# yhz0/SQLP

Measured on AMD Instinct MI355X. Metric: stage-2 subproblems/sec + cut-gen HBM GB/s on STORM, higher is better.
Workload: dtype f64

## Files before the change

### sqlp_amd/csrc/api.hip

```cpp
#include <hip/hip_runtime.h>
#include <algorithm>
#include <cmath>
#include <cstdarg>
#include <cstdio>
#include <cstdlib>
#include <cstring>
#include <string>
#include <vector>
#include <map>
#include <memory>
#include <thread>
#include <chrono>
#include "twosd_internal.h"
#include "twosd_ctx.h"

using namespace twosd;

static thread_local std::string g_err;

int twosd::fail(int code, const char *fmt, ...) {
    char buf[1024];
    va_list ap;
    va_start(ap, fmt);
    vsnprintf(buf, sizeof buf, fmt, ap);
// ... 203 lines not shown
}
template <typename T>
static int upload_big(twosd_ctx *c, T **d, const std::vector<T> &h) {
    return upload_big(c, d, h.data(), h.size());
}

static int reserve_selection(twosd_ctx *c, int P, int records) {
    int rc;
    if ((size_t)std::max(records, 1) > c->sel_code_cap) {
        dfree(c->d_sel_code);
        if ((rc = dalloc(&c->d_sel_code, 2 * (size_t)std::max(records, 1)))) return rc;
        c->sel_code_cap = std::max(records, 1);
    }
    if ((rc = dev_reserve(c, &c->d_sel_end, (size_t)P)) || (rc = dev_reserve(c, &c->d_sel_cinf, (size_t)P))) return rc;
    c->sel_cap_total = records;
    return TWOSD_OK;
}

template <typename T>
static int upload(T **d, const std::vector<T> &h) {
    int rc = dalloc(d, std::max<size_t>(h.size(), 1));
    if (rc) return rc;
    if (!h.empty()) HIPCHK(hipMemcpy(*d, h.data(), sizeof(T) * h.size(), hipMemcpyHostToDevice));
    return TWOSD_OK;
}

static void free_template(twosd_ctx *c) {
    dfree(c->d_colptr); dfree(c->d_rowidx); dfree(c->d_val); dfree(c->d_q); dfree(c->d_btype);
    dfree(c->d_fixedmask); dfree(c->d_ubmask);
    dfree(c->d_hb0); dfree(c->d_basic0);
    dfree(c->d_xbase); dfree(c->d_queue); dfree(c->d_lpstats);
    dfree(c->d_obj); dfree(c->d_pi); dfree(c->d_pi_rep); dfree(c->d_y); dfree(c->d_status); dfree(c->d_iters); dfree(c->d_ops); dfree(c->d_etan);
    dfree(c->d_dvtmp);
    dfree(c->d_bnnz); dfree(c->d_sel_cinf); dfree(c->d_sel_ptr); dfree(c->d_sel_code); c->sel_code_cap = 0; dfree(c->d_head_out); dfree(c->d_pool_pick); dfree(c->d_cpick); dfree(c->d_order); dfree(c->d_sort_tmp);
    dfree(c->d_cand); dfree(c->d_sel_key); dfree(c->d_sel_pkey); dfree(c->d_sel_ppick); c->sel_pcap = 0; c->key_cap = 0; c->pool_l1 = c->pool_ncand = 0; c->order_cap = 0; c->sort_tmp_bytes = 0; c->head_cap = 0; c->pick_cap = 0; c->pool.clear();
    dfree(c->d_dist_kind); dfree(c->d_dist_off); dfree(c->d_dist_val); dfree(c->d_dist_prob); dfree(c->d_dist_p0);
    dfree(c->d_dist_p1); dfree(c->d_dist_tmpl); c->has_dist = false;
    dfree(c->d_kslot); dfree(c->d_kix); dfree(c->d_kv); dfree(c->d_kcoef); c->k_valid = false;
    dfree(c->d_sel_end); dfree(c->d_kp); dfree(c->d_ke); dfree(c->d_kraw); dfree(c->d_xaux); c->xaux_cap = 0; c->sel_cap_total = 0;
    dfree(c->d_d0); dfree(c->d_eidx); dfree(c->d_evals); dfree(c->d_stamps);
    dfree(c->d_wcp); dfree(c->d_wcc); dfree(c->d_wcv); dfree(c->d_bcp); dfree(c->d_bci); dfree(c->d_bcv);
    dfree(c->d_brptr); dfree(c->d_brcol); dfree(c->d_brval);
    c->earena_slots = 0; c->earena_cap = 0;
    for (auto &e : c->epis) { dfree(e.d_dv); dfree(e.d_w); }
    c->epis.clear();
    c->out_cap = 0; c->dvtmp_cap = 0;
    dvs_free(c);
    cut_free(c);
    vkey_free(c);
    c->dcap.clear();
    dfree(c->d_vkey); c->vkey_cap = 0;
    dfree(c->d_bkey); c->bkey_cap = 0;
    dfree(c->d_refresh_sel); c->refresh_sel_cap = 0; c->box_epi = -1;
    dfree(c->d_eo_pb); dfree(c->d_eo_K); dfree(c->d_eo_off); dfree(c->d_eo_etap); dfree(c->d_eo_etaoff);
    dfree(c->d_eo_eidx); dfree(c->d_eo_evals); dfree(c->d_eo_used); c->eo_rows = c->eo_cap = 0; c->eo_kmax = 0;
    dfree(c->d_pg_scrow); dfree(c->d_pg_scoff); dfree(c->d_pg_scval); dfree(c->d_pg_ival); dfree(c->d_pg_irow); dfree(c->d_pg_ioff); dfree(c->d_pg_amax); dfree(c->d_pg_d0p); dfree(c->d_pg_cnt); dfree(c->d_pg_tot);
    dfree(c->d_pg_valid); dfree(c->d_pg_head0); dfree(c->d_pg_map); dfree(c->d_pg_off); dfree(c->d_pg_pos);
    dfree(c->d_rt_pack); dfree(c->d_gs_heads); dfree(c->d_gs_cnt); dfree(c->d_gs_tot); dfree(c->d_gs_valid);
    dfree(c->d_gs_irow); dfree(c->d_gs_ioff); dfree(c->d_gs_ival);
    if (c->d_gs_seg) { hipFree(c->d_gs_seg); c->d_gs_seg = nullptr; c->gs_seg_cap = 0; }
    c->rt_epi = -1; c->rt_nown = -1; c->rt_trained = false;
    if (c->pool_hb) { hipHostFree(c->pool_hb); c->pool_hb = nullptr; c->pool_hb_cap = 0; }
    c->has_template = c->has_basis = false;
}

extern "C" int twosd_destroy(twosd_ctx *c) {
    if (!c) return TWOSD_OK;
// ... 1907 lines not shown
            const size_t need = list ? (size_t)NL : (size_t)N;
            if (need > c->head_cap) {
                if ((rc = dalloc(&c->d_head_out, need * m))) return rc;
                c->head_cap = need;
            }
            H.head_out = c->d_head_out;
        }
        H.pi_by_pos = list ? 1 : 0;
        H.status = c->d_status; H.iters = c->d_iters; H.ops = c->d_ops; H.etan = c->d_etan;
        if (!c->d_lpstats && (rc = dalloc(&c->d_lpstats, 6))) return rc;
        if (!list) HIPCHK(hipMemsetAsync(c->d_lpstats + 5, 0, sizeof(unsigned long long), c->stream));
        H.retries = list ? nullptr : c->d_lpstats + 5;
        if (!c->d_stamps) {
            if ((rc = dalloc(&c->d_stamps, 16))) return rc;
            HIPCHK(hipMemset(c->d_stamps, 0, sizeof(unsigned long long) * 16));
        }
        H.stamps = c->d_stamps;
        H.npool = (int)c->pool.size();
        H.bnnz = c->d_bnnz;
        if (c->want_head && !list) {
            if ((size_t)N > c->head_cap) {
                if ((rc = dalloc(&c->d_head_out, (size_t)N * m))) return rc;
                c->head_cap = N;
            }
            H.head_out = c->d_head_out;
        }
        if (H.npool > 1) {
            if (!list && (size_t)N > c->pick_cap) {
                if ((rc = dalloc(&c->d_pool_pick, (size_t)N))) return rc;
                c->pick_cap = N;
            }
            H.pool_pick = c->d_pool_pick;
        }
        HIPCHK(hipEventRecord(c->ev[0], c->stream));
        if (list) {
            H.order = o.d_list;
        } else if (H.npool > 1) {
            if ((rc = select_pool(c, d_dv, N, c->d_pool_pick, 0))) return rc;
            H.order = c->d_order;
        }
        HIPCHK(hipEventRecord(c->ev[2], c->stream));
        HIPCHK(launch_hyper(R, CH, H, nblocks, hyper_lds_bytes(R, CH, kmax, c->k), c->stream));
        HIPCHK(hipEventRecord(c->ev[1], c->stream));
        HIPCHK(hipStreamSynchronize(c->stream));
        float ms = 0, ms_sel = 0;
        hipEventElapsedTime(&ms, c->ev[2], c->ev[1]);
        hipEventElapsedTime(&ms_sel, c->ev[0], c->ev[2]);
        c->t_us[0] = 1e3 * ms;
        c->t_us[4] = 1e3 * ms_sel;
        if (list) return TWOSD_OK;
        c->last_lp_N = N;
        c->last_lp_blocks = nblocks;
        c->last_ops_width = 1;
        return TWOSD_OK;
    }
}

__global__ void __launch_bounds__(256) lp_stats_kernel(int N, const int *__restrict__ its, const long long *__restrict__ ops,
                                                      const int *__restrict__ st, const int *__restrict__ etan,
                                                      unsigned long long *out) {
    __shared__ unsigned long long red[4][5];
    unsigned long long a = 0, b = 0, d = 0, e = 0;
    unsigned long long mx = 0;
    for (int s = blockIdx.x * blockDim.x + threadIdx.x; s < N; s += gridDim.x * blockDim.x) {
        a += (unsigned long long)its[s];
        b += (unsigned long long)ops[s];
        mx = its[s] > (int)mx ? (unsigned long long)its[s] : mx;
        d += st[s] != TWOSD_LP_OPTIMAL;
        e += (unsigned long long)etan[s];
    }
    for (int o = 32; o > 0; o >>= 1) {
        a += __shfl_down(a, o);
        b += __shfl_down(b, o);
        d += __shfl_down(d, o);
// ... 345 lines not shown
```

### sqlp_amd/csrc/lp_hyper.hip

```cpp
#include <hip/hip_runtime.h>
#include <math.h>
#include <type_traits>
#include "twosd_internal.h"
#include "wave_ops.h"

namespace twosd {

#define HTOL_P 1e-9
#define HTOL_D 1e-9
#define HTOL_PIV 1e-9
#define HPI_ZERO 1e-12


#ifdef TWOSD_STAMPS
#define STAMP_DECL unsigned long long st_acc[10] = {0, 0, 0, 0, 0, 0, 0, 0, 0, 0}; \
    unsigned long long st_last = __builtin_amdgcn_s_memtime();
#define STAMP(i)                                                      \
    {                                                                 \
        const unsigned long long t_ = __builtin_amdgcn_s_memtime();   \
        st_acc[i] += t_ - st_last;                                    \
        st_last = t_;                                                 \
    }
#define STAMP_FLUSH                                                                         \
    if (lane == 0 && P.stamps)                                                              \
// ... 152 lines not shown
    using Mask = typename std::conditional<(C > 32), uint64_t, uint32_t>::type;
    const int lane = threadIdx.x & 63;
    const int wid = threadIdx.x >> 6;
    constexpr int MP = 64 * R;
    constexpr int UD = 128 * R > 64 * C ? 128 * R : 64 * C;
    const int kmaxp = (P.kmax + 3) & ~3;
    const int ncol = P.n + P.m;
    char *slice = reinterpret_cast<char *>(lds_raw) + (size_t)wid * hyper_slice_bytes(R, C, P.kmax, P.k);
    double *ut = reinterpret_cast<double *>(slice);
    double *rho = ut + MP;
    double *alpha = ut;
    double *dvl = ut + UD;
    double *lstv = dvl + ((P.k + 1) & ~1);
    int *lsti = reinterpret_cast<int *>(lstv + 64);
    int *smark = lsti + 64;
    unsigned short *etap = reinterpret_cast<unsigned short *>(smark + 64);
    int *etaoff = reinterpret_cast<int *>(etap + kmaxp);

    const int m = P.m, n = P.n;
    const int slot_id = blockIdx.x * kWavesPerBlock + wid;
    int *eidx = P.eidx + (size_t)slot_id * P.ecap;
    double *evals = P.evals + (size_t)slot_id * P.ecap;
    const uint64_t fixedm = CP.fixedmask[lane];
    const uint64_t ubm = CP.ubmask[lane];

    for (int j = lane; j < UD; j += 64) ut[j] = 0.0;
    smark[lane] = 0;
    h_wave_sync();
    STAMP_DECL

    const int G = CP.qgroups;
    const int g0 = blockIdx.x % G;
    int gt = 0;
    auto group_of = [&](int gi) { return g0 + gi < G ? g0 + gi : g0 + gi - G; };
    auto claim_sync = [&]() -> int {
        for (; gt < G; ++gt) {
            const int g = group_of(gt);
            const int lo = (int)(((long long)P.N * g) / G), hi = (int)(((long long)P.N * (g + 1)) / G);
            int t = 0;
            if (lane == 0) t = atomicAdd(CP.queue + g * kQueueStride, 1);
            t = __builtin_amdgcn_readfirstlane(__shfl(t, 0));
            if (lo + t < hi) return lo + t;
        }
        return -1;
    };
    int q_nx = claim_sync();
    int s_nx = q_nx < 0 ? -1 : (CP.order ? __builtin_amdgcn_readfirstlane(CP.order[q_nx]) : q_nx);
    int pb_nx = (s_nx >= 0 && CP.npool > 1) ? __builtin_amdgcn_readfirstlane(CP.pool_pick[s_nx]) : 0;
    auto dv_fill = [&](int sn) {
        const double *dvs = CP.dv + (size_t)sn * P.k;
        for (int e = lane; e < P.k; e += 64) dvl[e] = CP.kcoef[e] * dvs[e];
    };
    const bool dv_pf = P.k <= 128;
    if (s_nx >= 0 && dv_pf) dv_fill(s_nx);
    for (;;) {
        if (q_nx < 0) break;
        const int qpos = q_nx;
        int s = s_nx;
        int pb = pb_nx;
        int t_claim = 0;
        if (lane == 0 && gt < G) t_claim = atomicAdd(CP.queue + group_of(gt) * kQueueStride, 1);

        if (!dv_pf) dv_fill(s);
        h_wave_sync();
        int lnx = lane;
        asm volatile("" : "+v"(lnx));
        double xB[R];
        float wd[R];
        int hb[R];
        double d[C];
        uint64_t bmask;
        const int *brptr, *bcp;
        int K = 0, it = 0, status = TWOSD_LP_OPTIMAL;
        int eoff = 0;
        unsigned nops = 0;
        for (int attempt = 0; attempt < 2; ++attempt) {
        {
            const auto *A = h_args();
            const int ln = lnx;
            brptr = A->brptr + (size_t)pb * (MP + 1);
            bcp = A->bcp + (size_t)pb * (MP + 1);
            const double *xb = A->xbase + (size_t)pb * MP;
            const double *kv = A->kv;
            const int *kix = A->kix;
            const int ksv = ln <= R ? A->kslot[pb * (R + 1) + ln] : 0;
            int eb[R], len[R];
            int w = 0;
#pragma unroll
            for (int t = 0; t < R; ++t) {
                eb[t] = __builtin_amdgcn_readlane(ksv, t);
                len[t] = __builtin_amdgcn_readlane(ksv, t + 1) - eb[t];
                w = len[t] > w ? len[t] : w;
                xB[t] = xb[64 * t + ln];
                hb[t] = A->hb0[(size_t)pb * MP + 64 * t + ln];
                wd[t] = 1.0f;
            }
            nops += (unsigned)(__builtin_amdgcn_readlane(ksv, R) - eb[0]) * 64u;
            for (int u0 = 0; u0 < w; u0 += XU) {
                double kvv[XU][R];
                int kiv[XU][R];
#pragma unroll
                for (int uu = 0; uu < XU; ++uu)
#pragma unroll
                    for (int t = 0; t < R; ++t) {
                        const int u = u0 + uu;
                        kvv[uu][t] = 0.0;
                        kiv[uu][t] = 0;
                        if (u < len[t]) {
                            kvv[uu][t] = kv[(size_t)(eb[t] + u) * 64 + ln];
                            kiv[uu][t] = kix[(size_t)(eb[t] + u) * 64 + ln];
                        }
                    }
#pragma unroll
                for (int uu = 0; uu < XU; ++uu)
#pragma unroll
                    for (int t = 0; t < R; ++t)
                        if (u0 + uu < len[t]) xB[t] = fma(kvv[uu][t], dvl[kiv[uu][t]], xB[t]);
            }
            uint64_t ub = ubm;
            asm volatile("" : "+v"(ub));
#pragma unroll
            for (int c = 0; c < C; ++c)
                d[c] = h_flip(A->d0[(size_t)pb * 64 * C + 64 * c + ln], ((ub >> c) & 1) << 63);
            bmask = A->basic0[pb * 64 + ln];
        }
        K = 0; status = TWOSD_LP_OPTIMAL; eoff = 0;
        if (lane == 0) etaoff[0] = 0;
        h_wave_sync();
        if (attempt == 0) {
            if (gt < G) {
                const int g = group_of(gt);
                const int hi = (int)(((long long)P.N * (g + 1)) / G), lo = (int)(((long long)P.N * g) / G);
                const int t = __builtin_amdgcn_readfirstlane(__shfl(t_claim, 0));
                if (lo + t < hi) q_nx = lo + t;
                else { ++gt; q_nx = claim_sync(); }
            } else {
                q_nx = -1;
            }
            if (q_nx >= 0) s_nx = CP.order ? CP.order[q_nx] : q_nx;
        }
        STAMP(0)

        auto eta_group = [&](int t0, int dir, int (&gi)[EG], double (&gv)[EG], int (&gn)[EG], int (&go)[EG]) {
#pragma unroll
            for (int g = 0; g < EG; ++g) {
                const int tt = t0 + dir * g;
                const bool ok = (tt >= 0) & (tt < K);
                const int tc = ok ? tt : 0;
                const int o0 = etaoff[tc], o1 = etaoff[tc + 1];
                go[g] = ok ? o0 : 0;
                gn[g] = ok ? o1 - o0 : 0;
                const bool mine = lane < gn[g];
                const int at = mine ? go[g] + lane : 0;
                const int ix = eidx[at];
                const double vx = evals[at];
                gi[g] = mine ? ix : 0;
                gv[g] = mine ? vx : 0.0;
            }
        };
        for (;;) {
            double bnum = 0.0, bden = 1.0, bdel = 0.0;
            int br = 0x7fffffff;
#pragma unroll
            for (int t = 0; t < R; ++t) {
                const int bt = hb[t] & 3;
                const bool inf = (hb[t] >= 0) & (((xB[t] < -HTOL_P) & (bt != BT_G)) | ((xB[t] > HTOL_P) & ((bt & 1) != 0)));
                if (__builtin_amdgcn_ballot_w64(inf) != 0 && inf) {
                    const double dl = xB[t];
                    const double num = dl * dl, den = (double)wd[t];
                    if (num * bden > bnum * den) { bnum = num; bden = den; br = 64 * t + lane; bdel = dl; }
                }
            }
            const ArgBest1 lr = warg_max1(bnum / bden, br, bdel);
// ... 8 lines not shown
                int p0 = 0, len = 0;
                double gr = 0.0;
                if (lane < nb) {
                    const int gi = lsti[lane];
                    gr = lstv[lane];
                    p0 = P.wcp[gi];
                    len = P.wcp[gi + 1] - p0;
                    alpha[n + gi] = P.btype[n + gi] == BT_G ? -gr : gr;
                }
                nops += h_seg_scatter(p0, len, gr, P.wcc, P.wcv, alpha, smark, lane) + nb;
                h_wave_sync();
            };
            int rp0 = 0, rlen = 65;
            if (K == 0) {
                rp0 = __builtin_amdgcn_readfirstlane(brptr[r]);
                rlen = __builtin_amdgcn_readfirstlane(brptr[r + 1]) - rp0;
            }
            if (rlen <= 64) {
                int gi = 0;
                double gr = 0.0;
                if (lane < rlen) {
                    gi = P.brcol[rp0 + lane];
                    gr = P.brval[rp0 + lane];
                }
                const uint64_t nzm = __ballot(gr != 0.0);
                if (gr != 0.0) {
                    const int pos = h_prefix_count(nzm);
                    lsti[pos] = gi;
                    lstv[pos] = gr;
                }
                nops += rlen;
                if (nzm != 0) price_batch(__popcll(nzm));
            } else {
                if (lane == (r & 63)) ut[r] = 1.0;
                h_wave_sync();
                const int gp0 = lane <= K ? (lane == 0 ? r : (int)etap[K - lane]) : -1;
                int bp0 = 0, bp1 = 0;
                if (gp0 >= 0) {
                    bp0 = brptr[gp0];
                    bp1 = brptr[gp0 + 1];
                }
                {
                    auto apply = [&](int tg, const int (&gi)[EG], const double (&gv)[EG], const int (&gn)[EG], const int (&go)[EG]) {
#pragma unroll
                        for (int g = 0; g < EG; ++g) {
                            const int tt = tg - g;
                            if (tt < 0) break;
                            const double ug = gv[g] != 0.0 ? ut[gi[g]] : 0.0;
                            if (gn[g] <= 64 && __builtin_amdgcn_ballot_w64(ug != 0.0) == 0) {
                                nops += gn[g];
                                continue;
                            }
                            double acc = ug * gv[g];
                            for (int e = 64 + lane; e < gn[g]; e += 64) acc = fma(ut[eidx[go[g] + e]], evals[go[g] + e], acc);
                            acc = wsum(acc);
                            nops += gn[g];
                            if (lane == 0) ut[etap[tt]] = acc;
                            h_wave_sync();
                        }
                    };
                    int ai[EG], an[EG], ao[EG], bi[EG], bn[EG], bo[EG];
                    double av[EG], bv[EG];
                    if (K <= 2 * EG) {
                        for (int tg = K - 1; tg >= 0; tg -= EG) {
                            eta_group(tg, -1, ai, av, an, ao);
                            apply(tg, ai, av, an, ao);
                        }
// ... 36 lines not shown
#pragma unroll
                for (int t = 0; t < R; ++t) rv[t] = rho[64 * t + lane];
                h_wave_sync();
#pragma unroll
                for (int t = 0; t < R; ++t) rho[64 * t + lane] = 0.0;
                h_wave_sync();
                uint64_t mk[R];
                int tot = 0;
#pragma unroll
                for (int t = 0; t < R; ++t) {
                    mk[t] = __ballot(rv[t] != 0.0);
                    tot += __popcll(mk[t]);
                }
                for (int b0 = 0; b0 < tot; b0 += 64) {
                    int base = -b0;
#pragma unroll
                    for (int t = 0; t < R; ++t) {
                        const int pos = base + h_prefix_count(mk[t]);
                        if (rv[t] != 0.0 && pos >= 0 && pos < 64) {
                            lsti[pos] = 64 * t + lane;
                            lstv[pos] = rv[t];
                        }
                        base += __popcll(mk[t]);
                    }
                    price_batch(tot - b0 < 64 ? tot - b0 : 64);
                }
            }
            h_wave_sync();
            STAMP(4)

            const uint64_t sgm = delta > 0 ? 0ull : (1ull << 63);
            const Mask cand = (Mask)~(bmask | fixedm);
            double bnu = INFINITY, bde = 1.0;
            Mask elm = 0, sel = 0, snz = 0;
            double apf = alpha[lane];
#pragma unroll
            for (int c = 0; c < C; ++c) {
                const double av = apf;
                if (c + 1 < C) apf = alpha[64 * (c + 1) + lane];
                const double a = h_flip(av, sgm);
                const bool el = (((cand >> c) & 1) != 0) & (a > HTOL_PIV);
                snz = h_uniform(snz | ((Mask)(__builtin_amdgcn_ballot_w64(av != 0.0) != 0) << c));
                if (__builtin_amdgcn_ballot_w64(el) != 0) {
                    sel |= (Mask)1 << c;
                    const double nu = d[c] + HTOL_D;
                    const bool better = el & (nu * bde < bnu * a);
                    bnu = better ? nu : bnu;
                    bde = better ? a : bde;
                    elm |= (Mask)el << c;
                }
                __builtin_amdgcn_sched_barrier(0);
            }
            const double thmax = wmin(bnu / bde);
            if (thmax == INFINITY) {
                status = TWOSD_LP_INFEASIBLE;
                h_wave_sync();
#pragma unroll
                for (int c = 0; c < C; ++c) alpha[64 * c + lane] = 0.0;
                break;
            }
            double bA = 0.0, bD = 0.0;
            int bq = 0x7fffffff;
            apf = alpha[lane];
#pragma unroll
            for (int c = 0; c < C; ++c) {
                const double av = apf;
// ... 160 lines not shown
            ++K;
            const int lh = h_get_row_i<R>(hb, r);
            const int leaving = lh >> 2;
            {
                const int ls = __builtin_amdgcn_readfirstlane(leaving >> 6), qs = __builtin_amdgcn_readfirstlane(q >> 6);
                const double dlv = (delta > 0) == ((lh & 3) == BT_G) ? thetaD : -thetaD;
                const bool lme = lane == (leaving & 63), qme = lane == (q & 63);
                H_SLOT_SWITCH(ls, C, {
                    double v = lme ? dlv : d[SL];
                    asm volatile("" : "+v"(v));
                    d[SL] = v;
                })
                H_SLOT_SWITCH(qs, C, {
                    double v = qme ? 0.0 : d[SL];
                    asm volatile("" : "+v"(v));
                    d[SL] = v;
                })
                if (lme) bmask &= ~(1ull << ls);
                if (qme) bmask |= 1ull << qs;
                {
                    const int nh = q * 4 + (int)P.btype[q];
                    const bool rme = lane == (r & 63);
                    H_SLOT_SWITCH(__builtin_amdgcn_readfirstlane(r >> 6), R, {
                        int v = rme ? nh : hb[SL];
                        asm volatile("" : "+v"(v));
                        hb[SL] = v;
                    })
                }
            }
            ++it;
            h_wave_sync();
            STAMP(8)
        }
        if (attempt == 0 && q_nx >= 0) {
            s_nx = __builtin_amdgcn_readfirstlane(s_nx);
            if (CP.npool > 1) pb_nx = CP.pool_pick[s_nx];
        }
        if (status == TWOSD_LP_OPTIMAL || pb == 0 || !CP.retry) break;
        if (lane == 0 && CP.retries) atomicAdd(CP.retries, 1ull);
        pb = 0;
        }
        double dvn0 = 0.0, dvn1 = 0.0, kcn0 = 0.0, kcn1 = 0.0;
        if (dv_pf && q_nx >= 0) {
            const auto *A = h_args();
            const double *dvs = A->dv + (size_t)s_nx * P.k;
            if (lane < P.k) { dvn0 = dvs[lane]; kcn0 = A->kcoef[lane]; }
            if (lane + 64 < P.k) { dvn1 = dvs[lane + 64]; kcn1 = A->kcoef[lane + 64]; }
        }

        double objv = NAN;
        if (status == TWOSD_LP_OPTIMAL) {
            const double *qc = CP.q;
            double qv[R];
#pragma unroll
            for (int t = 0; t < R; ++t) {
                const int j = hb[t] >> 2;
                qv[t] = qc[(hb[t] >= 0 && j < n) ? j : 0];
            }
            double ob = 0.0;
#pragma unroll
            for (int t = 0; t < R; ++t) {
                const int j = hb[t] >> 2;
                ob = (hb[t] >= 0 && j < n) ? fma(qv[t], xB[t], ob) : ob;
            }
            objv = wsum(ob);
            if (CP.vkey) {
                uint64_t ub = ubm;
                int lane = threadIdx.x & 63;
                asm volatile("" : "+v"(ub), "+v"(lane));
                auto dk = [&](int c) -> double {
                    const int j = 64 * c + lane;
                    const bool slack = (j >= n) & (j < ncol) & (((bmask >> c) & 1) == 0);
                    return slack ? h_flip(d[c], ((ub >> c) & 1) << 63) : 0.0;
                };
                double pm = 0.0;
#pragma unroll
                for (int c = 0; c < C; ++c) pm = fmax(pm, fabs(dk(c)));
                pm = wmax(pm);
                const double zt = CP.key_zero * (1.0 + pm);
                unsigned long long h = 0;
#pragma unroll
                for (int c = 0; c < C; ++c) {
                    const int j = 64 * c + lane;
                    if (j >= n && j < ncol) {
                        const double dc = dk(c);
                        const double v = fabs(dc) <= zt ? 0.0 : dc;
                        const unsigned long long b = ((unsigned long long)__double_as_longlong(v) + (1ull << 28)) >> 29;
                        h += mix64(((unsigned long long)(j - n) << 35) | b);
                    }
                }
#pragma unroll
                for (int o = 32; o > 0; o >>= 1) h += __shfl_xor(h, o);
                if (lane == 0) CP.vkey[s] = h;
            }
        }
        if constexpr (FULL) {
        if (status == TWOSD_LP_OPTIMAL && (P.pi || P.y)) {
            const double *qc = CP.q;
#pragma unroll
            for (int t = 0; t < R; ++t) {
                const int j = hb[t] >> 2;
                const bool bq = hb[t] >= 0 && j < n;
                const double qj = qc[bq ? j : 0];
                ut[64 * t + lane] = bq ? qj : 0.0;
            }
            h_wave_sync();
            for (int tt = K - 1; tt >= 0; --tt) {
                const int off = etaoff[tt], nnz = etaoff[tt + 1] - off;
                double acc = 0.0;
                for (int e = lane; e < nnz; e += 64) acc = fma(ut[eidx[off + e]], evals[off + e], acc);
                acc = wsum(acc);
                nops += nnz;
                if (lane == 0) ut[etap[tt]] = acc;
                h_wave_sync();
            }
            double pv[R];
            double pmax = 0.0;
#pragma unroll
            for (int t = 0; t < R; ++t) {
                const int cc = 64 * t + lane;
                const int e0 = cc < m ? bcp[cc] : 0, e1 = cc < m ? bcp[cc + 1] : 0;
                double a = 0.0;
#pragma unroll TWOSD_REC_UNROLL
                for (int e = e0; e < e1; ++e) a = fma(ut[P.bci[e]], P.bcv[e], a);
                pv[t] = a;
                pmax = fmax(pmax, fabs(a));
// ... 37 lines not shown
                if (64 * t + lane < m) P.head_out[ho + 64 * t + lane] = hb[t] >> 2;
        }
        if (P.bkey && status == TWOSD_LP_OPTIMAL) {
            unsigned long long h = 0;
#pragma unroll
            for (int t = 0; t < R; ++t)
                if (64 * t + lane < m) h += mix64((unsigned long long)(hb[t] >> 2));
#pragma unroll
            for (int o = 32; o > 0; o >>= 1) h += __shfl_xor(h, o);
            if (lane == 0) P.bkey[s] = h;
        }
        if (P.eo_K) {
            const int erow = P.pi_by_pos ? qpos : s;
            unsigned long long off64 = 0;
            if (lane == 0 && status == TWOSD_LP_OPTIMAL) off64 = atomicAdd(P.eo_used, (unsigned long long)eoff);
            off64 = __shfl(off64, 0);
            const bool ok = status == TWOSD_LP_OPTIMAL && off64 + (unsigned long long)eoff <= (unsigned long long)P.eo_cap;
            const int off = ok ? (int)off64 : 0;
            if (ok) {
                for (int e = lane; e < eoff; e += 64) {
                    P.eo_eidx[off + e] = eidx[e];
                    P.eo_evals[off + e] = evals[e];
                }
                for (int t = lane; t < K; t += 64) P.eo_etap[(size_t)erow * P.kmax + t] = etap[t];
                for (int t = lane; t <= K; t += 64) P.eo_etaoff[(size_t)erow * (P.kmax + 1) + t] = etaoff[t];
            }
            if (lane == 0) {
                P.eo_K[erow] = ok ? K : -1;
                P.eo_off[erow] = off;
                P.eo_pb[erow] = pb;
            }
        }
        }
        if (lane == 0) {
            CP.obj[s] = objv;
            CP.status[s] = status;
            CP.iters[s] = it;
            if (CP.ops) CP.ops[s] = (long long)nops;
            if (CP.etan) CP.etan[s] = eoff;
            if (CP.npool > 1) CP.pool_pick[s] = pb;
        }
        if (dv_pf && q_nx >= 0) {
            if (lane < P.k) dvl[lane] = kcn0 * dvn0;
            if (lane + 64 < P.k) dvl[lane + 64] = kcn1 * dvn1;
        }
        h_wave_sync();
        pb_nx = __builtin_amdgcn_readfirstlane(pb_nx);
        STAMP(9)
    }
    STAMP_FLUSH
}

__device__ __forceinline__ float h_viol_f(float x, float cw) { return x > 1e-9f ? x + cw : 0.0f; }

constexpr int kSelWaves = 16;
#ifndef TWOSD_SEL_B
#define TWOSD_SEL_B 16
#endif
constexpr int kSelB = TWOSD_SEL_B;
typedef float sel_f2 __attribute__((ext_vector_type(2)));
constexpr int kSelTile = 128;
__device__ __forceinline__ sel_f2 h_viol_f2(sel_f2 x, float cw) {
    sel_f2 r;
    r.x = h_viol_f(x.x, cw);
    r.y = h_viol_f(x.y, cw);
    return r;
}
template <typename RowOf>
__device__ __forceinline__ void h_stage_pairs(float *dvt, const double *__restrict__ dv, const double *__restrict__ kcoef,
                                              int k, int nv, RowOf srow) {
    for (int idx = threadIdx.x; idx < kSelTile * k; idx += 64 * kSelWaves) {
        const int sl = idx / k, e = idx - sl * k;
        dvt[2 * (e * 65 + (sl & 63)) + (sl >> 6)] = sl < nv ? (float)(kcoef[e] * dv[(size_t)srow(sl) * k + e]) : 0.0f;
    }
}
__device__ __forceinline__ const sel_f2 *h_pair_addr(const sel_f2 *dvt2, int off, int lane8) {
    int o;
    asm("v_max_i32 %0, %1, 0" : "=v"(o) : "s"(off));
    return reinterpret_cast<const sel_f2 *>(reinterpret_cast<const char *>(dvt2) + o + lane8);
}
// ... 194 lines not shown
    }
    if (bc >= 0) pick[s] = cand[(size_t)pick[s] * ncand + bc];
}

static int sel_split(int N, int items) {
    if (getenv("TWOSD_SEL_NOSPLIT")) return 1;
    const int nb = (N + kSelTile - 1) / kSelTile;
    int g = (1024 + nb - 1) / nb;
    g = std::min(g, std::max(1, items / kSelWaves));
    return std::max(1, std::min(g, 64));
}
int pool_select_split(int N, int npool) { return sel_split(N, npool); }
int pool_refine_split(int N, int ncand) { return sel_split(N, ncand); }

hipError_t launch_pool_refine(const PoolRefineParams &p, hipStream_t s) {
    if (p.N <= 0 || p.ncand <= 0) return hipSuccess;
    const int G = p.pkey ? pool_refine_split(p.N, p.ncand) : 1;
    hipLaunchKernelGGL(pool_refine_kernel, dim3((p.N + kSelTile - 1) / kSelTile, G), dim3(64 * kSelWaves), pool_select_lds_bytes(p.k), s, p);
    if (G > 1) hipLaunchKernelGGL(pool_refine_merge_kernel, dim3((p.N + 255) / 256), dim3(256), 0, s, p.N, G, p.ncand, p.pkey, p.pci, p.cand, p.pick);
    return hipGetLastError();
}

size_t pool_select_lds_bytes(int k) { return (size_t)4 * 65 * (kSelTile / 64) * (size_t)std::max(k, 1); }

hipError_t launch_pool_select(const PoolSelParams &p, hipStream_t s) {
    if (p.N <= 0) return hipSuccess;
    const int nb = (p.N + kSelTile - 1) / kSelTile;
    const int G = p.pkey ? pool_select_split(p.N, p.npool) : 1;
    hipLaunchKernelGGL(pool_select_kernel, dim3(nb, G), dim3(64 * kSelWaves), pool_select_lds_bytes(p.k), s, p);
    if (G > 1) hipLaunchKernelGGL(pool_select_merge_kernel, dim3((p.N + 255) / 256), dim3(256), 0, s, p.N, G, p.pkey, p.ppick, p.pick, p.key);
    return hipGetLastError();
}

static const int kHR[] = {1, 2, 4, 9, 16};
static const int kHC[] = {2, 4, 8, 14, 16, 28, 32, 64};

int hyper_rows_per_lane(int m) {
    for (int R : kHR)
        if (m <= 64 * R) return R;
    return -1;
}
int hyper_cols_per_lane(int ncols) {
    for (int C : kHC)
        if (ncols <= 64 * C) return C;
    return -1;
}

template <int R, int C>
static hipError_t hl(const HyperParams &p, int nb, size_t lds, hipStream_t s) {
    if (p.pi || p.y || p.head_out || p.bkey || p.eo_K)
        hipLaunchKernelGGL((lp_hyper_kernel<R, C, true>), dim3(nb), dim3(256), lds, s, p);
    else
        hipLaunchKernelGGL((lp_hyper_kernel<R, C, false>), dim3(nb), dim3(256), lds, s, p);
    return hipGetLastError();
}
template <int R, int C>
static int ho(size_t lds) {
    int nb = 0, nb2 = 0;
    if (hipOccupancyMaxActiveBlocksPerMultiprocessor(&nb, lp_hyper_kernel<R, C, true>, 256, lds) != hipSuccess) return 1;
    if (hipOccupancyMaxActiveBlocksPerMultiprocessor(&nb2, lp_hyper_kernel<R, C, false>, 256, lds) != hipSuccess) return 1;
    nb = std::min(nb, nb2);
    return nb > 0 ? nb : 1;
}

#ifdef HYP_DEV_STORM_ONLY
#define HYPER_C_SWITCH(R, FN, ...)                  \
// ... 42 lines not shown
```

### sqlp_amd/csrc/twosd_ctx.h

```cpp
#pragma once
#include <hip/hip_runtime.h>
#include <stdint.h>
#include <map>
#include <vector>
#include "twosd_internal.h"

namespace twosd {

struct EpiDevice {
    double *d_dv = nullptr;
    double *d_w = nullptr;
    size_t dv_cap = 0, w_cap = 0;
    int count = 0;
    double total_weight = 0.0;
    std::vector<double> w_host;
};

struct PoolBasis {
    std::vector<int> head;
    std::vector<double> Binv;
    std::vector<double> pi0;
    std::vector<int> rptr, rcol;
    std::vector<double> rval;
    bool dev_only = false;
// ... 27 lines not shown
    uint64_t *d_basic0 = nullptr;
    double *d_xbase = nullptr;
    std::vector<twosd::PoolBasis> pool;
    float *d_sel_cinf = nullptr;
    int *d_sel_ptr = nullptr, *d_sel_code = nullptr;
    int *d_sel_end = nullptr;
    int *d_kp = nullptr, *d_ke = nullptr;
    double *d_kraw = nullptr;
    double *d_xaux = nullptr;
    size_t xaux_cap = 0;
    int64_t sel_cap_total = 0;
    size_t sel_code_cap = 0;
    int64_t sel_nnz = 0, sel_rows = 0;
    float sel_cw = 0.0f;
    std::vector<double> dist_mad;
    std::vector<double> sel_lo, sel_hi;
    int *d_bnnz = nullptr;
    int *d_head_out = nullptr, *d_pool_pick = nullptr;
    size_t head_cap = 0, pick_cap = 0;
    int pool_l1 = 0, pool_ncand = 0;
    int *d_cand = nullptr;
    std::vector<int> cand_p1, cand_pf;
    int cand_pl1 = 0, cand_pnc = 0;
    bool cand_pending = false;
    int *d_cpick = nullptr;
    float *d_sel_key = nullptr;
    float *d_sel_pkey = nullptr;
    int *d_sel_ppick = nullptr;
    size_t sel_pcap = 0;
    size_t key_cap = 0;
    int *d_order = nullptr;
    char *d_sort_tmp = nullptr;
    size_t order_cap = 0, sort_tmp_bytes = 0;
    bool want_head = false;
    bool prep_valid = false;
    bool k_valid = false;
    double *d_kcoef = nullptr;
    std::vector<double> prep_x;
    size_t xbase_cap = 0, kcoef_cap = 0;
    int CH = 0;
    int *d_kslot = nullptr, *d_kix = nullptr;
    double *d_kv = nullptr, *d_d0 = nullptr;
    int *d_bcp = nullptr, *d_bci = nullptr;
    double *d_bcv = nullptr;
    int *d_wcp = nullptr, *d_wcc = nullptr;
    double *d_wcv = nullptr;
    int *d_brptr = nullptr, *d_brcol = nullptr;
    double *d_brval = nullptr;
    int *d_eidx = nullptr;
    double *d_evals = nullptr;
    size_t earena_slots = 0;
    int earena_cap = 0;
    int64_t last_iterlimit = 0;
    int64_t b0_nnz = 0;
    unsigned long long *d_stamps = nullptr;
    int last_ops_width = 1;
    int *d_queue = nullptr;
    unsigned long long *d_lpstats = nullptr;
    double *d_obj = nullptr, *d_pi = nullptr, *d_y = nullptr;
    int *d_status = nullptr, *d_iters = nullptr;
    long long *d_ops = nullptr;
    int *d_etan = nullptr;
    int64_t last_eta_entries = 0;
    int64_t last_retries = 0;
    int64_t last_ops_sum = 0;
    int out_cap = 0;
// ... 91 lines not shown
```

### sqlp_amd/csrc/twosd_internal.h

```cpp
#pragma once
#include <hip/hip_runtime.h>
#include <stdint.h>
#include <string>
#include <vector>
#include "twosd_hip.h"

namespace twosd {

constexpr int kWave = 64;
constexpr int kWavesPerBlock = 4;
constexpr int kMaxColsPerLane = 64;

enum : int { BT_Y = 0, BT_G = 1, BT_L = 2, BT_E = 3 };


constexpr int kQueueStride = 32;
constexpr int kMaxQueueGroups = 64;
struct HyperParams {
    int m, n, k, N, kmax, ecap;
    int kcap;
    int retry;
    const int *colptr, *rowidx; const double *val;
    const double *q; const int8_t *btype;
    const int *wcp, *wcc; const double *wcv;
    const int *bcp, *bci; const double *bcv;
    const int *brptr, *brcol; const double *brval;
    const int *kslot, *kix; const double *kv;
    const double *kcoef;
    const double *xbase;
    const double *d0;
    const int *hb0;
    const uint64_t *basic0, *fixedmask, *ubmask;
    const double *dv;
    int *eidx; double *evals;
    int *queue;
    int qgroups;
    double *obj, *pi, *y;
    int *status, *iters;
    long long *ops;
    int *etan;
    unsigned long long *retries;
    unsigned long long *stamps;
    int npool;
    const int *bnnz;
    int *head_out;
    int *pool_pick;
    const int *order;
    unsigned long long *vkey;
    double key_zero;
    int pi_by_pos;
    unsigned long long *bkey;
    int *eo_pb, *eo_K, *eo_off, *eo_etap, *eo_etaoff;
    int *eo_eidx; double *eo_evals;
    unsigned long long *eo_used; long long eo_cap;
};

struct PgArgs {
    int m, n, MP, CH, R9, k, kmax, npool_old;
    const int *colptr, *rowidx; const double *val, *q; const int8_t *btype; const int *pos_row;
    const int *bcp0, *bci0; const double *bcv0;
    const int *eo_pb, *eo_K, *eo_off, *eo_etap, *eo_etaoff, *eo_eidx; const double *eo_evals;
    const int *head0, *heads;
    const int *src_row;
    const int *gheads;
    int a0;
    double *amax;
    int *nzc, *keptc;
    int *nztot;
    const long long *inter_off;
    int *inter_row; double *inter_val;
    int *rowcnt, *erowcnt;
    int *tot;
    int *valid;
    long long sc_cap;
    int *sc_row, *sc_off; double *sc_val;
};
struct PgFill {
    int P0, P;
    const int *map;
    const int *off;
    int sel_total;
// ... 19 lines not shown
    int N, k, npool;
    const double *dv;
    const double *kcoef;
    const float *cinf;
    const int *sptr, *send;
    const int2 *rec;
    int *pick;
    float cw;
    float *key;
    float *pkey; int *ppick;
};
struct PoolRefineParams {
    int N, k, ncand;
    const double *dv, *kcoef;
    const float *cinf;
    const int *sptr, *send;
    const int2 *rec;
    const int *order, *cand;
    int *pick;
    const float *key;
    float cw;
    float *pkey; int *pci;
};
hipError_t launch_pool_refine(const PoolRefineParams &p, hipStream_t s);
size_t pool_select_lds_bytes(int k);
int pool_select_split(int N, int npool);
int pool_refine_split(int N, int ncand);
hipError_t sort_by_pool(const int *pick, int *order, int N, int npool, void *tmp, size_t *tmp_bytes, hipStream_t s);
hipError_t launch_pool_select(const PoolSelParams &p, hipStream_t s);
size_t hyper_lds_bytes(int R, int C, int kmax, int k);
int hyper_rows_per_lane(int m);
int hyper_cols_per_lane(int ncols);
hipError_t launch_hyper(int R, int C, const HyperParams &p, int nblocks, size_t lds, hipStream_t s);
int hyper_max_blocks_per_cu(int R, int C, int kmax, int k);


struct SampleParams {
    int N, k;
    unsigned long long seed, first_index;
    const int *kind;
    const int *off;
    const double *val, *prob;
    const double *p0, *p1;
    const double *tmpl;
    double *out;
};
hipError_t launch_sample(const SampleParams &S, hipStream_t st);

struct HostLP {
    int m = 0, n = 0;
    std::vector<int> colptr, rowidx;
    std::vector<double> val, q;
    std::vector<char> sense;
};
bool dense_inverse(int m, const std::vector<double> &A, std::vector<double> &Ainv);
void basis_matrix(const HostLP &L, const std::vector<int> &head, std::vector<double> &B);
int setup_solve(const HostLP &L, const std::vector<double> &b, std::vector<int> &head, double &obj,
                int &iters, std::string &err);
double basis_dual_infeasibility(const HostLP &L, const std::vector<int> &head,
                                const std::vector<double> &Binv, std::vector<double> &pi0);
void compose_binv(int m, const std::vector<int> &rptr0, const std::vector<int> &rcol0, const std::vector<double> &rval0,
                  int K, const int *etap, const int *etaoff, const int *eidx, const double *evals, std::vector<int> &rptr,
                  std::vector<int> &rcol, std::vector<double> &rval);
double sparse_dual_infeasibility(const HostLP &L, const std::vector<int> &head, const std::vector<double> &pi0);
double sparse_basis_residual(const HostLP &L, const std::vector<int> &head, const std::vector<int> &rptr,
                             const std::vector<int> &rcol, const std::vector<double> &rval, int probes);
// ... 12 lines not shown
```

Before: 16.19 million.

## Precompute queue records and pipeline next-subproblem claim and prefetch in hyper LP kernel

Adds a small kernel that packs each queue position's scenario index and pool pick into an int2 record, so the LP kernel reads one record instead of chasing order then pool_pick. The hyper kernel now claims the work item two steps ahead and prefetches the next basis's kslot row into LDS. It also loads xbase, hb0, d0 and basic0 before the ELL x_B update, and rewrites that update with branch-free predicated loads separated by sched barriers. Output writes are batched through readfirstlane'd pointers, and a TWOSD_DEBUG ELL-width report is added. The extra launch and more live registers may hurt occupancy.

```diff
diff --git a/sqlp_amd/csrc/api.hip b/sqlp_amd/csrc/api.hip
--- a/sqlp_amd/csrc/api.hip
+++ b/sqlp_amd/csrc/api.hip
@@ -259,7 +259,7 @@
     dfree(c->d_xbase); dfree(c->d_queue); dfree(c->d_lpstats);
     dfree(c->d_obj); dfree(c->d_pi); dfree(c->d_pi_rep); dfree(c->d_y); dfree(c->d_status); dfree(c->d_iters); dfree(c->d_ops); dfree(c->d_etan);
     dfree(c->d_dvtmp);
-    dfree(c->d_bnnz); dfree(c->d_sel_cinf); dfree(c->d_sel_ptr); dfree(c->d_sel_code); c->sel_code_cap = 0; dfree(c->d_head_out); dfree(c->d_pool_pick); dfree(c->d_cpick); dfree(c->d_order); dfree(c->d_sort_tmp);
+    dfree(c->d_bnnz); dfree(c->d_sel_cinf); dfree(c->d_sel_ptr); dfree(c->d_sel_code); c->sel_code_cap = 0; dfree(c->d_head_out); dfree(c->d_pool_pick); dfree(c->d_cpick); dfree(c->d_order); dfree(c->d_sort_tmp); dfree(c->d_qrec); c->qrec_cap = 0;
     dfree(c->d_cand); dfree(c->d_sel_key); dfree(c->d_sel_pkey); dfree(c->d_sel_ppick); c->sel_pcap = 0; c->key_cap = 0; c->pool_l1 = c->pool_ncand = 0; c->order_cap = 0; c->sort_tmp_bytes = 0; c->head_cap = 0; c->pick_cap = 0; c->pool.clear();
     dfree(c->d_dist_kind); dfree(c->d_dist_off); dfree(c->d_dist_val); dfree(c->d_dist_prob); dfree(c->d_dist_p0);
     dfree(c->d_dist_p1); dfree(c->d_dist_tmpl); c->has_dist = false;
@@ -2233,14 +2233,39 @@
             }
             H.pool_pick = c->d_pool_pick;
         }
+        if (!list && c->d_kslot && getenv("TWOSD_DEBUG")) {
+            std::vector<int> ks((size_t)H.npool * (R + 1));
+            HIPCHK(hipMemcpy(ks.data(), c->d_kslot, sizeof(int) * ks.size(), hipMemcpyDeviceToHost));
+            std::vector<int> ws(H.npool);
+            double mean = 0;
+            for (int p = 0; p < H.npool; ++p) {
+                int w = 0;
+                for (int t = 0; t < R; ++t) w = std::max(w, ks[(size_t)p * (R + 1) + t + 1] - ks[(size_t)p * (R + 1) + t]);
+                ws[p] = w;
+                mean += w;
+            }
+            std::sort(ws.begin(), ws.end());
+            fprintf(stderr, "LP start: ELL width w over %d bases: min %d, median %d, mean %.2f, p90 %d, max %d\n", H.npool, ws.front(),
+                    ws[ws.size() / 2], mean / H.npool, ws[ws.size() * 9 / 10], ws.back());
+        }
         HIPCHK(hipEventRecord(c->ev[0], c->stream));
+        const int *order = nullptr;
         if (list) {
-            H.order = o.d_list;
+            order = o.d_list;
         } else if (H.npool > 1) {
             if ((rc = select_pool(c, d_dv, N, c->d_pool_pick, 0))) return rc;
-            H.order = c->d_order;
+            order = c->d_order;
         }
         HIPCHK(hipEventRecord(c->ev[2], c->stream));
+        if (order || H.npool > 1) {
+            if ((size_t)NL > c->qrec_cap) {
+                const size_t cap = std::max<size_t>(NL, 1024);
+                if ((rc = dalloc(&c->d_qrec, cap))) return rc;
+                c->qrec_cap = cap;
+            }
+            HIPCHK(launch_queue_records(order, H.npool > 1 ? c->d_pool_pick : nullptr, c->d_qrec, NL, c->stream));
+            H.qrec = c->d_qrec;
+        }
         HIPCHK(launch_hyper(R, CH, H, nblocks, hyper_lds_bytes(R, CH, kmax, c->k), c->stream));
         HIPCHK(hipEventRecord(c->ev[1], c->stream));
         HIPCHK(hipStreamSynchronize(c->stream));
diff --git a/sqlp_amd/csrc/lp_hyper.hip b/sqlp_amd/csrc/lp_hyper.hip
--- a/sqlp_amd/csrc/lp_hyper.hip
+++ b/sqlp_amd/csrc/lp_hyper.hip
@@ -208,21 +208,42 @@
     const int G = CP.qgroups;
     const int g0 = blockIdx.x % G;
     int gt = 0;
+    int q_lo = 0, q_hi = 0;
     auto group_of = [&](int gi) { return g0 + gi < G ? g0 + gi : g0 + gi - G; };
+    auto range_set = [&]() {
+        const int g = group_of(gt);
+        q_lo = (int)(((long long)P.N * g) / G);
+        q_hi = (int)(((long long)P.N * (g + 1)) / G);
+    };
+    auto claim_issue = [&]() -> int {
+        int t = 0;
+        if (lane == 0 && gt < G) t = atomicAdd(CP.queue + group_of(gt) * kQueueStride, 1);
+        return t;
+    };
     auto claim_sync = [&]() -> int {
         for (; gt < G; ++gt) {
-            const int g = group_of(gt);
-            const int lo = (int)(((long long)P.N * g) / G), hi = (int)(((long long)P.N * (g + 1)) / G);
-            int t = 0;
-            if (lane == 0) t = atomicAdd(CP.queue + g * kQueueStride, 1);
-            t = __builtin_amdgcn_readfirstlane(__shfl(t, 0));
-            if (lo + t < hi) return lo + t;
+            range_set();
+            const int t = __builtin_amdgcn_readfirstlane(claim_issue());
+            if (q_lo + t < q_hi) return q_lo + t;
         }
         return -1;
     };
+    auto claim_resolve = [&](int t_claim) -> int {
+        if (gt >= G) return -1;
+        const int t = __builtin_amdgcn_readfirstlane(t_claim);
+        if (q_lo + t < q_hi) return q_lo + t;
+        ++gt;
+        return claim_sync();
+    };
     int q_nx = claim_sync();
-    int s_nx = q_nx < 0 ? -1 : (CP.order ? __builtin_amdgcn_readfirstlane(CP.order[q_nx]) : q_nx);
-    int pb_nx = (s_nx >= 0 && CP.npool > 1) ? __builtin_amdgcn_readfirstlane(CP.pool_pick[s_nx]) : 0;
+    int q_n2 = q_nx >= 0 ? claim_resolve(claim_issue()) : -1;
+    int s_nx = q_nx, pb_nx = 0;
+    if (q_nx >= 0 && CP.qrec) {
+        const int2 rc = CP.qrec[q_nx];
+        s_nx = __builtin_amdgcn_readfirstlane(rc.x);
+        pb_nx = __builtin_amdgcn_readfirstlane(rc.y);
+    }
+    if (q_nx >= 0 && lane <= R) lsti[lane] = CP.kslot[pb_nx * (R + 1) + lane];
     auto dv_fill = [&](int sn) {
         const double *dvs = CP.dv + (size_t)sn * P.k;
         for (int e = lane; e < P.k; e += 64) dvl[e] = CP.kcoef[e] * dvs[e];
@@ -234,9 +255,7 @@
         const int qpos = q_nx;
         int s = s_nx;
         int pb = pb_nx;
-        int t_claim = 0;
-        if (lane == 0 && gt < G) t_claim = atomicAdd(CP.queue + group_of(gt) * kQueueStride, 1);
-
+        q_nx = q_n2;
         if (!dv_pf) dv_fill(s);
         h_wave_sync();
         int lnx = lane;
@@ -257,9 +276,29 @@
             brptr = A->brptr + (size_t)pb * (MP + 1);
             bcp = A->bcp + (size_t)pb * (MP + 1);
             const double *xb = A->xbase + (size_t)pb * MP;
+            const int *hbp = A->hb0 + (size_t)pb * MP;
+            const double *d0p = A->d0 + (size_t)pb * 64 * C;
             const double *kv = A->kv;
             const int *kix = A->kix;
-            const int ksv = ln <= R ? A->kslot[pb * (R + 1) + ln] : 0;
+            int ksv = 0;
+            if (attempt == 0) {
+                if (ln <= R) ksv = lsti[ln];
+            } else if (ln <= R) {
+                ksv = A->kslot[pb * (R + 1) + ln];
+            }
+            double d0r[C];
+#pragma unroll
+            for (int t = 0; t < R; ++t) {
+                xB[t] = xb[64 * t + ln];
+                hb[t] = hbp[64 * t + ln];
+                wd[t] = 1.0f;
+            }
+#pragma unroll
+            for (int c = 0; c < C; ++c) d0r[c] = d0p[64 * c + ln];
+            bmask = A->basic0[pb * 64 + ln];
+            const bool has_rec = A->qrec != nullptr;
+            int2 rcn = make_int2(0, 0);
+            if (attempt == 0 && q_nx >= 0 && has_rec) rcn = A->qrec[q_nx];
             int eb[R], len[R];
             int w = 0;
 #pragma unroll
@@ -267,54 +306,46 @@
                 eb[t] = __builtin_amdgcn_readlane(ksv, t);
                 len[t] = __builtin_amdgcn_readlane(ksv, t + 1) - eb[t];
                 w = len[t] > w ? len[t] : w;
-                xB[t] = xb[64 * t + ln];
-                hb[t] = A->hb0[(size_t)pb * MP + 64 * t + ln];
-                wd[t] = 1.0f;
             }
             nops += (unsigned)(__builtin_amdgcn_readlane(ksv, R) - eb[0]) * 64u;
             for (int u0 = 0; u0 < w; u0 += XU) {
-                double kvv[XU][R];
+                double kvv[XU][R], dg[XU][R];
                 int kiv[XU][R];
 #pragma unroll
                 for (int uu = 0; uu < XU; ++uu)
 #pragma unroll
                     for (int t = 0; t < R; ++t) {
                         const int u = u0 + uu;
-                        kvv[uu][t] = 0.0;
-                        kiv[uu][t] = 0;
-                        if (u < len[t]) {
-                            kvv[uu][t] = kv[(size_t)(eb[t] + u) * 64 + ln];
-                            kiv[uu][t] = kix[(size_t)(eb[t] + u) * 64 + ln];
-                        }
+                        const size_t e = u < len[t] ? (size_t)(eb[t] + u) : 0;
+                        kvv[uu][t] = kv[e * 64 + ln];
+                        kiv[uu][t] = kix[e * 64 + ln];
                     }
+                __builtin_amdgcn_sched_barrier(0);
 #pragma unroll
                 for (int uu = 0; uu < XU; ++uu)
 #pragma unroll
-                    for (int t = 0; t < R; ++t)
-                        if (u0 + uu < len[t]) xB[t] = fma(kvv[uu][t], dvl[kiv[uu][t]], xB[t]);
+                    for (int t = 0; t < R; ++t) dg[uu][t] = dvl[kiv[uu][t]];
+                __builtin_amdgcn_sched_barrier(0);
+#pragma unroll
+                for (int uu = 0; uu < XU; ++uu)
+#pragma unroll
+                    for (int t = 0; t < R; ++t) {
+                        const double v = fma(kvv[uu][t], dg[uu][t], xB[t]);
+                        xB[t] = u0 + uu < len[t] ? v : xB[t];
+                    }
             }
             uint64_t ub = ubm;
             asm volatile("" : "+v"(ub));
 #pragma unroll
-            for (int c = 0; c < C; ++c)
-                d[c] = h_flip(A->d0[(size_t)pb * 64 * C + 64 * c + ln], ((ub >> c) & 1) << 63);
-            bmask = A->basic0[pb * 64 + ln];
+            for (int c = 0; c < C; ++c) d[c] = h_flip(d0r[c], ((ub >> c) & 1) << 63);
+            if (attempt == 0 && q_nx >= 0) {
+                s_nx = has_rec ? __builtin_amdgcn_readfirstlane(rcn.x) : q_nx;
+                pb_nx = has_rec ? __builtin_amdgcn_readfirstlane(rcn.y) : 0;
+            }
         }
         K = 0; status = TWOSD_LP_OPTIMAL; eoff = 0;
         if (lane == 0) etaoff[0] = 0;
         h_wave_sync();
-        if (attempt == 0) {
-            if (gt < G) {
-                const int g = group_of(gt);
-                const int hi = (int)(((long long)P.N * (g + 1)) / G), lo = (int)(((long long)P.N * g) / G);
-                const int t = __builtin_amdgcn_readfirstlane(__shfl(t_claim, 0));
-                if (lo + t < hi) q_nx = lo + t;
-                else { ++gt; q_nx = claim_sync(); }
-            } else {
-                q_nx = -1;
-            }
-            if (q_nx >= 0) s_nx = CP.order ? CP.order[q_nx] : q_nx;
-        }
         STAMP(0)
 
         auto eta_group = [&](int t0, int dir, int (&gi)[EG], double (&gv)[EG], int (&gn)[EG], int (&go)[EG]) {
@@ -389,7 +420,11 @@
                 nops += rlen;
                 if (nzm != 0) price_batch(__popcll(nzm));
             } else {
-                if (lane == (r & 63)) ut[r] = 1.0;
+                {
+                    double one = 1.0;
+                    asm volatile("" : "+v"(one));
+                    if (lane == (r & 63)) ut[r] = one;
+                }
                 h_wave_sync();
                 const int gp0 = lane <= K ? (lane == 0 ? r : (int)etap[K - lane]) : -1;
                 int bp0 = 0, bp1 = 0;
@@ -492,6 +527,7 @@
             const uint64_t sgm = delta > 0 ? 0ull : (1ull << 63);
             const Mask cand = (Mask)~(bmask | fixedm);
             double bnu = INFINITY, bde = 1.0;
+            asm volatile("" : "+v"(bde));
             Mask elm = 0, sel = 0, snz = 0;
             double apf = alpha[lane];
 #pragma unroll
@@ -718,23 +754,25 @@
             h_wave_sync();
             STAMP(8)
         }
-        if (attempt == 0 && q_nx >= 0) {
-            s_nx = __builtin_amdgcn_readfirstlane(s_nx);
-            if (CP.npool > 1) pb_nx = CP.pool_pick[s_nx];
-        }
         if (status == TWOSD_LP_OPTIMAL || pb == 0 || !CP.retry) break;
         if (lane == 0 && CP.retries) atomicAdd(CP.retries, 1ull);
         pb = 0;
         }
         double dvn0 = 0.0, dvn1 = 0.0, kcn0 = 0.0, kcn1 = 0.0;
-        if (dv_pf && q_nx >= 0) {
+        int ksn = 0, t_claim = 0;
+        if (q_nx >= 0) {
             const auto *A = h_args();
-            const double *dvs = A->dv + (size_t)s_nx * P.k;
-            if (lane < P.k) { dvn0 = dvs[lane]; kcn0 = A->kcoef[lane]; }
-            if (lane + 64 < P.k) { dvn1 = dvs[lane + 64]; kcn1 = A->kcoef[lane + 64]; }
+            t_claim = claim_issue();
+            if (lane <= R) ksn = A->kslot[pb_nx * (R + 1) + lane];
+            if (dv_pf) {
+                const double *dvs = A->dv + (size_t)s_nx * P.k;
+                if (lane < P.k) { dvn0 = dvs[lane]; kcn0 = A->kcoef[lane]; }
+                if (lane + 64 < P.k) { dvn1 = dvs[lane + 64]; kcn1 = A->kcoef[lane + 64]; }
+            }
         }
 
         double objv = NAN;
+        unsigned long long keyv = 0;
         if (status == TWOSD_LP_OPTIMAL) {
             const double *qc = CP.q;
             double qv[R];
@@ -750,6 +788,18 @@
                 ob = (hb[t] >= 0 && j < n) ? fma(qv[t], xB[t], ob) : ob;
             }
             objv = wsum(ob);
+        }
+        q_n2 = -1;
+        if (q_nx >= 0) {
+            q_n2 = claim_resolve(t_claim);
+            if (lane <= R) lsti[lane] = ksn;
+            if (dv_pf) {
+                if (lane < P.k) dvl[lane] = kcn0 * dvn0;
+                if (lane + 64 < P.k) dvl[lane + 64] = kcn1 * dvn1;
+            }
+        }
+        h_wave_sync();
+        if (status == TWOSD_LP_OPTIMAL) {
             if (CP.vkey) {
                 uint64_t ub = ubm;
                 int lane = threadIdx.x & 63;
@@ -777,7 +827,7 @@
                 }
 #pragma unroll
                 for (int o = 32; o > 0; o >>= 1) h += __shfl_xor(h, o);
-                if (lane == 0) CP.vkey[s] = h;
+                keyv = h;
             }
         }
         if constexpr (FULL) {
@@ -881,20 +931,24 @@
             }
         }
         }
-        if (lane == 0) {
-            CP.obj[s] = objv;
-            CP.status[s] = status;
-            CP.iters[s] = it;
-            if (CP.ops) CP.ops[s] = (long long)nops;
-            if (CP.etan) CP.etan[s] = eoff;
-            if (CP.npool > 1) CP.pool_pick[s] = pb;
-        }
-        if (dv_pf && q_nx >= 0) {
-            if (lane < P.k) dvl[lane] = kcn0 * dvn0;
-            if (lane + 64 < P.k) dvl[lane + 64] = kcn1 * dvn1;
+        {
+            const auto *A = h_args();
+            double *const o_obj = A->obj;
+            int *const o_status = A->status, *const o_iters = A->iters, *const o_etan = A->etan, *const o_pick = A->pool_pick;
+            long long *const o_ops = A->ops;
+            unsigned long long *const o_key = A->vkey;
+            const int su = __builtin_amdgcn_readfirstlane(s);
+            if (lane == 0) {
+                o_obj[su] = objv;
+                o_status[su] = status;
+                o_iters[su] = it;
+                if (o_ops) o_ops[su] = (long long)nops;
+                if (o_etan) o_etan[su] = eoff;
+                if (o_pick) o_pick[su] = pb;
+                if (o_key && status == TWOSD_LP_OPTIMAL) o_key[su] = keyv;
+            }
         }
         h_wave_sync();
-        pb_nx = __builtin_amdgcn_readfirstlane(pb_nx);
         STAMP(9)
     }
     STAMP_FLUSH
@@ -1155,6 +1209,19 @@
     return hipGetLastError();
 }
 
+__global__ void __launch_bounds__(256) queue_records_kernel(int N, const int *__restrict__ order, const int *__restrict__ pick,
+                                                           int2 *__restrict__ qrec) {
+    const int q = blockIdx.x * blockDim.x + threadIdx.x;
+    if (q >= N) return;
+    const int s = order ? order[q] : q;
+    qrec[q] = make_int2(s, pick ? pick[s] : 0);
+}
+hipError_t launch_queue_records(const int *order, const int *pick, int2 *qrec, int N, hipStream_t s) {
+    if (N <= 0) return hipSuccess;
+    hipLaunchKernelGGL(queue_records_kernel, dim3((N + 255) / 256), dim3(256), 0, s, N, order, pick, qrec);
+    return hipGetLastError();
+}
+
 static const int kHR[] = {1, 2, 4, 9, 16};
 static const int kHC[] = {2, 4, 8, 14, 16, 28, 32, 64};
 
diff --git a/sqlp_amd/csrc/twosd_ctx.h b/sqlp_amd/csrc/twosd_ctx.h
--- a/sqlp_amd/csrc/twosd_ctx.h
+++ b/sqlp_amd/csrc/twosd_ctx.h
@@ -83,6 +83,8 @@
     int *d_order = nullptr;
     char *d_sort_tmp = nullptr;
     size_t order_cap = 0, sort_tmp_bytes = 0;
+    int2 *d_qrec = nullptr;
+    size_t qrec_cap = 0;
     bool want_head = false;
     bool prep_valid = false;
     bool k_valid = false;
diff --git a/sqlp_amd/csrc/twosd_internal.h b/sqlp_amd/csrc/twosd_internal.h
--- a/sqlp_amd/csrc/twosd_internal.h
+++ b/sqlp_amd/csrc/twosd_internal.h
@@ -35,18 +35,19 @@
     int *eidx; double *evals;
     int *queue;
     int qgroups;
-    double *obj, *pi, *y;
+    double *obj;
     int *status, *iters;
     long long *ops;
     int *etan;
+    int *pool_pick;
+    unsigned long long *vkey;
+    double *pi, *y;
     unsigned long long *retries;
     unsigned long long *stamps;
     int npool;
     const int *bnnz;
     int *head_out;
-    int *pool_pick;
-    const int *order;
-    unsigned long long *vkey;
+    const int2 *qrec;
     double key_zero;
     int pi_by_pos;
     unsigned long long *bkey;
@@ -132,6 +133,7 @@
 int hyper_rows_per_lane(int m);
 int hyper_cols_per_lane(int ncols);
 hipError_t launch_hyper(int R, int C, const HyperParams &p, int nblocks, size_t lds, hipStream_t s);
+hipError_t launch_queue_records(const int *order, const int *pick, int2 *qrec, int N, hipStream_t s);
 int hyper_max_blocks_per_cu(int R, int C, int kmax, int k);
 
 
```

Result: faster. 16.59 million, median of 6 (+2.5%).
